# PaddlePaddle/PaddleScience

Hardware: AMD Instinct MI355X
Metric: collocation-points/sec (PDE residual+grad) (higher is better)
Workload: dtype f32; 1 GPU; Allen-Cahn 1D+t, MLP 2->64x4->1 tanh, 100k collocation pts per GPU, residual+MSE-mean+grad+Adam (BASELINE.json configs[1]); points_per_gpu=100000, parallelism=dp1, dp_step=fused tile kernel + tail kernel (sums, Adam, fragments)

## Files before the change

### paddlescience_amd/_lib.py

```python
from __future__ import annotations

import ctypes as C
import os
from typing import List, Optional, Sequence

MAX_IN, MAX_DIRS, MAX_OUT, MAX_HIDDEN, MAX_PROG, MAX_RES, MAX_AUX = 8, 4, 8, 16, 128, 8, 16

ACT = {"tanh": 0, "silu": 1, "sin": 2, "sigmoid": 3, "cos": 4, "gelu": 5, "swish": 6, "stan": 7, "relu": 8, "leaky_relu": 9,
       "elu": 10, "selu": 11, "identity": 12}
PARAM_ACTS = ("swish", "stan")
SIREN_W0 = 30.0
LINEAR_PLAIN, LINEAR_WEIGHT_NORM, LINEAR_RWF, LINEAR_FOURIER, LINEAR_BROADCAST = range(5)
LINEAR_PADDED = 100
EMBED_NONE, EMBED_PERIOD, EMBED_STREAMS = 0, 1, 2

(OP_LD_IN, OP_LD_U, OP_LD_AUX, OP_CONST, OP_ADD, OP_SUB, OP_MUL, OP_DIV, OP_NEG, OP_POW, OP_SIN, OP_COS,
 OP_TANH, OP_EXP, OP_LOG, OP_SQRT, OP_ABS, OP_SINH, OP_COSH, OP_TAN, OP_MAX, OP_MIN, OP_SIGN, OP_HEAVISIDE,
 OP_DETACH, OP_ASIN, OP_ACOS, OP_ATAN, OP_ATAN2, OP_ASINH, OP_ACOSH, OP_ATANH, OP_ERF, OP_LGAMMA, OP_CEIL, OP_FLOOR,
 OP_LD_PARAM, OP_COUNT) = range(38)
MAX_EPARAM = 8
MTL_MAX_LOSSES = 8
MTL_PCGRAD, MTL_GRAM_ONLY = 0, 1
STEP_KEEP_FRAGMENTS = 1


class MlpDesc(C.Structure):
    _fields_ = [
        ("d_raw", C.c_int32), ("n_hidden", C.c_int32), ("width", C.c_int32), ("d_out", C.c_int32),
        ("activation", C.c_int32), ("skip_connection", C.c_int32), ("n1", C.c_int32), ("n2", C.c_int32),
        ("embed", C.c_int32 * MAX_IN), ("omega", C.c_float * MAX_IN), ("dirs", (C.c_float * MAX_IN) * MAX_DIRS),
        ("act_scale", C.c_float), ("fourier_half", C.c_int32), ("n3", C.c_int32), ("n4", C.c_int32),
    ]


class SpectralDesc(C.Structure):
    _fields_ = [(n, C.c_int32) for n in ("batch", "c_in", "c_out", "h", "wf", "modes_x", "modes_y")]


class PwVirtual(C.Structure):
    _fields_ = [("mode", C.c_int32), ("K0", C.c_int32), ("x0", C.c_void_p), ("W0", C.c_void_p), ("b0", C.c_void_p)]


class ReduceSeg(C.Structure):
    _fields_ = [("partials", C.c_void_p), ("out", C.c_void_p), ("rows", C.c_int64), ("cols", C.c_int64), ("accumulate", C.c_int32)]


class LinearJob(C.Structure):
    _fields_ = [("kind", C.c_int32), ("fin", C.c_int32), ("fout", C.c_int32)] + [(n, C.c_void_p) for n in (
        "v", "g", "b", "W", "b_out", "gW", "gb", "gv", "gg", "gb_out")]


class ModMlpDesc(C.Structure):
    _fields_ = [(n, C.c_int32) for n in ("n_hidden", "width", "d_out", "activation")]


class SpinnGridDesc(C.Structure):
    _fields_ = [("n", C.c_int32 * 3), ("rank", C.c_int32), ("cu", C.c_float), ("cxx", C.c_float), ("cyy", C.c_float),
                ("czz", C.c_float), ("scale", C.c_float)]


SPINN_MAX_JET = 16


class SpinnJetDesc(C.Structure):
    _fields_ = [("n", C.c_int32 * 3), ("rank", C.c_int32), ("nq", C.c_int32), ("ord", (C.c_int32 * 3) * SPINN_MAX_JET)]


class PirateEmbedDesc(C.Structure):
    _fields_ = [("d_raw", C.c_int32), ("d0", C.c_int32), ("half", C.c_int32), ("n1", C.c_int32), ("n2", C.c_int32),
                ("embed", C.c_int32 * MAX_IN), ("omega", C.c_float * MAX_IN), ("dirs", (C.c_float * MAX_IN) * MAX_DIRS),
                ("N", C.c_int64), ("NP", C.c_int64)]


PIRATE_ACT, PIRATE_GATE, PIRATE_RES = 0, 1, 2


ONET_MAX_J = 3


class OnetHeadDesc(C.Structure):
    _fields_ = [("J", C.c_int32), ("p", C.c_int32), ("n_out", C.c_int32), ("n1", C.c_int32), ("n2", C.c_int32),
                ("act", C.c_int32), ("N", C.c_int64), ("NP", C.c_int64)]


class Fno1dLayerDesc(C.Structure):
    _fields_ = ([(k, C.c_void_p) for k in ("A1", "T", "A2", "X2", "bias", "ip_src", "ip_i0", "ip_t", "ia_src", "ia_first", "dact_v",
                                           "v", "out", "hw2", "hb2", "hy")]
                + [(k, C.c_int64) for k in ("a1_bs", "a2_rs", "a2_cs", "x2_bs", "ip_bs", "ia_bs", "dv_bs", "o_bs")]
                + [(k, C.c_int32) for k in ("ldt", "x2_ld", "x2_len", "ip_ld", "ia_ld", "dv_ld", "o_ld", "act", "B", "R", "K1", "K2",
                                            "Lc", "Lout")])


class LnoTriDesc(C.Structure):
    _fields_ = ([("n", C.c_int32 * 3), ("m", C.c_int32 * 3)] + [(k, C.c_int32) for k in (
        "nb", "ncp", "nc2", "C", "pair_cp", "pair_c2", "conj_t", "coef_b", "coef_cp", "coef_c2", "mult_conj")]
        + [("gscale", C.c_float)])


class Instr(C.Structure):
    _fields_ = [("op", C.c_int32), ("a", C.c_int32), ("b", C.c_int32), ("c", C.c_float)]


class Residual(C.Structure):
    _fields_ = [("value", C.c_int32), ("label", C.c_int32), ("weight", C.c_int32), ("area", C.c_int32),
                ("scale", C.c_float), ("kind", C.c_int32), ("scale_param", C.c_int32)]


class EpilogueDesc(C.Structure):
    _fields_ = [
        ("n_instr", C.c_int32), ("n_res", C.c_int32), ("n_streams", C.c_int32), ("n_in", C.c_int32),
        ("n_aux", C.c_int32), ("prog", Instr * MAX_PROG), ("res", Residual * MAX_RES),
    ]


class AdamArgs(C.Structure):
    _fields_ = [("m", C.c_void_p), ("v", C.c_void_p), ("lr", C.c_float), ("beta1", C.c_float), ("beta2", C.c_float),
                ("eps", C.c_float), ("grad_scale", C.c_float), ("step_t", C.c_int64)]


_HERE = os.path.dirname(os.path.abspath(__file__))
DEFAULT_LIB = os.environ.get("PPSCI_HIP_LIB") or os.path.join(_HERE, "libppsci_hip.so")
_lib: Optional[C.CDLL] = None
_injected = False

_SYMBOLS = {
    "ppsci_last_error": (C.c_char_p, []),
    "ppsci_is_device_build": (C.c_int, []),
    "ppsci_check_device": (C.c_int, []),
    "ppsci_linear_multi": (C.c_int, [C.c_int, C.POINTER(LinearJob), C.c_int, C.c_void_p]),
    "ppsci_reduce_rows_multi": (C.c_int, [C.c_int, C.POINTER(ReduceSeg), C.c_void_p]),
    "ppsci_reduce_rows_multi_adam": (C.c_int, [C.c_int, C.POINTER(ReduceSeg), C.c_int64, C.c_void_p, C.c_void_p, C.c_void_p,
                                               C.c_void_p, C.c_float, C.c_float, C.c_float, C.c_float, C.c_int64, C.c_float,
                                               C.c_void_p]),
    "ppsci_release_fragments": (None, [C.c_void_p]),
    "ppsci_set_max_grid": (None, [C.c_int]),
    "ppsci_set_wide_min_nb": (None, [C.c_int]),
    "ppsci_set_bwd_accum": (None, [C.c_int]),
    "ppsci_set_bwd_layerwise": (None, [C.c_int]),
    "ppsci_comm_unique_id": (C.c_int, [C.c_void_p]),
    "ppsci_comm_init": (C.c_int, [C.c_int, C.c_int, C.c_void_p]),
    "ppsci_comm_world_size": (C.c_int, []),
    "ppsci_allreduce_sum": (C.c_int, [C.c_void_p, C.c_int64, C.c_void_p]),
    "ppsci_allgather": (C.c_int, [C.c_void_p, C.c_void_p, C.c_int64, C.c_void_p]),
    "ppsci_comm_destroy": (C.c_int, []),
    "ppsci_param_count": (C.c_int64, [C.POINTER(MlpDesc)]),
    "ppsci_stash_bytes": (C.c_int64, [C.POINTER(MlpDesc), C.c_int64]),
    "ppsci_bwd_partial_rows": (C.c_int64, [C.POINTER(MlpDesc), C.c_int64]),
    "ppsci_bwd_workspace_bytes": (C.c_int64, [C.POINTER(MlpDesc), C.c_int64]),
    "ppsci_epilogue_partial_rows": (C.c_int64, [C.c_int64]),
    "ppsci_taylor_fwd": (C.c_int, [C.POINTER(MlpDesc), C.c_void_p, C.c_int64, C.POINTER(C.c_void_p), C.c_void_p,
                                   C.c_void_p, C.c_void_p]),
    "ppsci_epilogue": (C.c_int, [C.POINTER(EpilogueDesc), C.c_int64, C.POINTER(C.c_void_p), C.c_void_p,
                                 C.POINTER(C.c_void_p), C.c_void_p, C.c_void_p, C.c_void_p, C.c_void_p]),
    "ppsci_epilogue_losses": (C.c_int, [C.POINTER(EpilogueDesc), C.c_int64, C.POINTER(C.c_void_p), C.c_void_p,
                                        C.POINTER(C.c_void_p), C.c_void_p, C.c_void_p, C.c_void_p, C.c_void_p,
                                        C.c_void_p, C.c_void_p, C.c_void_p, C.c_void_p]),
    "ppsci_epilogue_params": (C.c_int, [C.POINTER(EpilogueDesc), C.c_int64, C.POINTER(C.c_void_p), C.c_void_p,
                                        C.POINTER(C.c_void_p), C.c_void_p, C.c_void_p, C.c_void_p, C.c_void_p,
                                        C.c_void_p, C.c_void_p]),
    "ppsci_taylor_bwd": (C.c_int, [C.POINTER(MlpDesc), C.c_void_p, C.c_int64, C.POINTER(C.c_void_p), C.c_void_p,
                                   C.c_void_p, C.c_void_p, C.c_void_p, C.c_void_p]),
    "ppsci_taylor_bwd_ws": (C.c_int, [C.POINTER(MlpDesc), C.c_void_p, C.c_int64, C.POINTER(C.c_void_p), C.c_void_p,
                                      C.c_void_p, C.c_void_p, C.c_int64, C.c_void_p, C.c_void_p]),
    "ppsci_dense_matvec": (C.c_int, [C.c_int64, C.c_int64, C.c_void_p, C.c_void_p, C.c_void_p, C.c_float, C.c_int, C.c_void_p,
                                     C.c_void_p]),
    "ppsci_csr_matvec": (C.c_int, [C.c_int64, C.c_int64, C.c_int64, C.c_void_p, C.c_void_p, C.c_void_p, C.c_void_p, C.c_void_p,
                                   C.c_float, C.c_void_p, C.c_void_p]),
    "ppsci_reduce_rows": (C.c_int, [C.c_void_p, C.c_int64, C.c_int64, C.c_void_p, C.c_int, C.c_void_p]),
    "ppsci_taylor_step_workspace_bytes": (C.c_int64, [C.POINTER(MlpDesc), C.POINTER(EpilogueDesc), C.c_int64]),
    "ppsci_taylor_step_kind": (C.c_int, [C.POINTER(MlpDesc), C.POINTER(EpilogueDesc), C.c_int64]),
    "ppsci_set_fused_step": (None, [C.c_int]),
    "ppsci_set_step_tail": (None, [C.c_int]),
    "ppsci_set_tail_split": (None, [C.c_int]),
    "ppsci_set_fast_program": (None, [C.c_int]),
    "ppsci_taylor_step_run_ex": (C.c_int, [C.c_void_p, C.c_int, C.POINTER(AdamArgs), C.c_void_p, C.c_int]),
    "ppsci_taylor_step_plan_apply": (C.c_int, [C.c_void_p, C.POINTER(AdamArgs), C.c_void_p]),
    "ppsci_set_static_program": (None, [C.c_int]),
    "ppsci_epilogue_predecode": (C.c_int, [C.POINTER(EpilogueDesc), C.POINTER(C.c_uint32), C.POINTER(C.c_int)]),
    "ppsci_taylor_step_plan_static": (C.c_int, [C.c_void_p, C.POINTER(C.c_char_p)]),
    "ppsci_set_fused_specialised": (None, [C.c_int]),
    "ppsci_taylor_step_plan_specialised": (C.c_int, [C.c_void_p]),
    "ppsci_set_fused_keep_planes": (None, [C.c_int]),
    "ppsci_taylor_step_plan_keep_planes": (C.c_int, [C.c_void_p]),
    "ppsci_taylor_step_plan": (C.c_void_p, [C.POINTER(MlpDesc), C.POINTER(EpilogueDesc), C.c_void_p, C.c_int64,
                                            C.POINTER(C.c_void_p), C.POINTER(C.c_void_p), C.c_void_p, C.c_void_p, C.c_void_p,
                                            C.c_void_p, C.c_void_p, C.c_int64, C.c_void_p, C.c_void_p]),
    "ppsci_taylor_step_run": (C.c_int, [C.c_void_p, C.c_int, C.POINTER(AdamArgs), C.c_void_p]),
    "ppsci_taylor_step_plan_set_scales": (C.c_int, [C.c_void_p, C.POINTER(EpilogueDesc)]),
    "ppsci_taylor_step_run_main": (C.c_int, [C.c_void_p, C.c_void_p]),
    "ppsci_taylor_step_plan_free": (None, [C.c_void_p]),
    "ppsci_taylor_step": (C.c_int, [C.POINTER(MlpDesc), C.POINTER(EpilogueDesc), C.c_void_p, C.c_int64, C.POINTER(C.c_void_p),
                                    C.POINTER(C.c_void_p), C.c_void_p, C.c_void_p, C.c_void_p, C.c_void_p, C.c_void_p,
                                    C.c_int64, C.c_void_p, C.c_void_p, C.c_int, C.POINTER(AdamArgs), C.c_void_p]),
    "ppsci_spectral_conv2d_fwd": (C.c_int, [C.POINTER(SpectralDesc), C.c_void_p, C.c_void_p, C.c_void_p, C.c_void_p,
                                            C.c_void_p]),
    "ppsci_spectral_conv2d_bwd": (C.c_int, [C.POINTER(SpectralDesc), C.c_void_p, C.c_void_p, C.c_void_p, C.c_void_p,
                                            C.c_void_p, C.c_void_p, C.c_void_p, C.c_void_p]),
    "ppsci_spectral_conv2d_bwd_real": (C.c_int, [C.POINTER(SpectralDesc), C.c_void_p, C.c_void_p, C.c_void_p, C.c_void_p,
                                                 C.c_void_p, C.c_void_p, C.c_void_p, C.c_float, C.c_int, C.c_void_p]),
    "ppsci_spectral_conv2d_fwd_scaled": (C.c_int, [C.POINTER(SpectralDesc), C.c_void_p, C.c_void_p, C.c_void_p, C.c_void_p,
                                                   C.c_float, C.c_int, C.c_void_p]),
    "ppsci_spectral_conv2d_bwd_real_scaled": (C.c_int, [C.POINTER(SpectralDesc), C.c_void_p, C.c_void_p, C.c_void_p,
                                                        C.c_void_p, C.c_void_p, C.c_void_p, C.c_void_p, C.c_float, C.c_int,
                                                        C.c_float, C.c_int, C.c_void_p]),
    "ppsci_dft2_kept_supported": (C.c_int, [C.c_int] * 4),
    "ppsci_dft2_kept_fwd": (C.c_int, [C.c_int] * 6 + [C.c_void_p] * 3),
    "ppsci_dft2_kept_inv": (C.c_int, [C.c_int] * 6 + [C.c_void_p] * 3),
    "ppsci_dft2_kept_inv_stats": (C.c_int, [C.c_int] * 6 + [C.c_void_p] * 3 + [C.c_int, C.c_void_p, C.c_void_p]),
    "ppsci_fno_tail_fwd_ex": (C.c_int, [C.c_int] * 5 + [C.c_float] + [C.c_void_p] * 9 + [C.c_int] * 5 + [C.c_void_p, C.c_void_p]),
    "ppsci_fno_tail_bwd_ex": (C.c_int, [C.c_int] * 5 + [C.c_void_p] * 13 + [C.c_int] * 4 + [C.c_void_p] * 3),
    "ppsci_spectral_conv2d_fwd_kept": (C.c_int, [C.POINTER(SpectralDesc)] + [C.c_void_p] * 4 + [C.c_float, C.c_void_p]),
    "ppsci_spectral_conv2d_inv_kept_ex": (C.c_int, [C.POINTER(SpectralDesc)] + [C.c_int] * 6 + [C.c_void_p, C.c_void_p, C.c_void_p, C.c_float,
                                                    C.c_void_p, C.c_void_p, C.c_void_p, C.c_void_p]),
    "ppsci_spectral_conv2d_inv_kept_supported": (C.c_int, [C.c_int] * 6),
    "ppsci_spectral_conv2d_inv_kept": (C.c_int, [C.POINTER(SpectralDesc), C.c_int, C.c_int, C.c_int, C.c_void_p, C.c_void_p,
                                                 C.c_void_p, C.c_float, C.c_void_p, C.c_void_p, C.c_void_p, C.c_void_p]),
    "ppsci_spectral_conv2d_bwd_kept": (C.c_int, [C.POINTER(SpectralDesc)] + [C.c_void_p] * 7 + [C.c_float, C.c_int, C.c_float,
                                                                                                 C.c_void_p]),
    "ppsci_fft2d_r2c": (C.c_int, [C.c_int, C.c_int, C.c_int, C.c_void_p, C.c_void_p, C.c_void_p]),
    "ppsci_fft2d_c2r": (C.c_int, [C.c_int, C.c_int, C.c_int, C.c_void_p, C.c_void_p, C.c_void_p]),
    "ppsci_pw_conv": (C.c_int, [C.c_int, C.c_int, C.c_int, C.c_int, C.c_void_p, C.c_void_p, C.c_int, C.c_void_p, C.c_void_p,
                                C.c_int, C.c_void_p, C.c_void_p, C.c_void_p]),
    "ppsci_pw_conv_v": (C.c_int, [C.c_int, C.c_int, C.c_int, C.c_int, C.c_void_p, C.POINTER(PwVirtual), C.c_void_p, C.c_int,
                                  C.c_void_p, C.c_void_p, C.POINTER(PwVirtual), C.c_int, C.c_void_p, C.c_void_p, C.c_void_p]),
    "ppsci_fno_proj_hidden_grad": (C.c_int, [C.c_int, C.c_int, C.c_int, C.c_int, C.c_void_p, C.c_void_p, C.c_void_p, C.c_void_p, C.c_void_p]),
    "ppsci_fno_lift0_wgrad": (C.c_int, [C.c_int, C.c_int, C.c_int, C.c_int, C.c_int, C.c_void_p, C.c_void_p, C.c_void_p, C.c_void_p,
                                        C.c_void_p, C.c_void_p, C.c_void_p, C.c_void_p, C.c_int64, C.c_void_p, C.c_int64, C.c_void_p]),
    "ppsci_pw_conv_wgrad_v": (C.c_int, [C.c_int, C.c_int, C.c_int, C.c_int, C.c_void_p, C.POINTER(PwVirtual), C.c_void_p,
                                        C.c_void_p, C.c_void_p, C.c_int64, C.c_void_p]),
    "ppsci_set_pw_pixels_per_lane": (None, [C.c_int]),
    "ppsci_pw_conv_wgrad_chunks": (C.c_int64, [C.c_int, C.c_int]),
    "ppsci_fno_lift0_wgrad_chunks": (C.c_int64, [C.c_int, C.c_int]),
    "ppsci_pw_conv_wgrad": (C.c_int, [C.c_int, C.c_int, C.c_int, C.c_int, C.c_void_p, C.c_void_p, C.c_void_p, C.c_void_p,
                                      C.c_void_p]),
    "ppsci_pad2d": (C.c_int, [C.c_int] * 8 + [C.c_void_p, C.c_void_p, C.c_void_p]),
    "ppsci_dft2_kept_from_supported": (C.c_int, [C.c_int] * 4),
    "ppsci_dft2_kept_fwd_from": (C.c_int, [C.c_int] * 7 + [C.c_void_p, C.c_void_p, C.c_void_p]),
    "ppsci_dft2_kept_inv_from": (C.c_int, [C.c_int] * 7 + [C.c_void_p, C.c_void_p, C.c_void_p]),
    "ppsci_sht_supported": (C.c_int, [C.c_int] * 4),
    "ppsci_sht_analysis": (C.c_int, [C.c_int] * 5 + [C.c_void_p] * 5),
    "ppsci_sht_synthesis": (C.c_int, [C.c_int] * 5 + [C.c_void_p] * 5),
    "ppsci_sht_contract": (C.c_int, [C.c_int] * 5 + [C.c_void_p] * 3 + [C.c_int, C.c_void_p, C.c_void_p]),
    "ppsci_sht_contract_wgrad": (C.c_int, [C.c_int] * 5 + [C.c_void_p] * 5),
    "ppsci_spectrum_resize": (C.c_int, [C.c_int] * 7 + [C.c_void_p, C.c_void_p, C.c_void_p]),
    "ppsci_resample2d_supported": (C.c_int, [C.c_int] * 4),
    "ppsci_resample2d": (C.c_int, [C.c_int] * 5 + [C.c_void_p] * 4 + [C.c_int, C.c_void_p]),
    "ppsci_field_loss_sums": (C.c_int, [C.c_int] * 4 + [C.c_float, C.c_float, C.c_int, C.c_int] + [C.c_void_p] * 4),
    "ppsci_field_loss_finish": (C.c_int, [C.c_int, C.c_int, C.c_float, C.c_float] + [C.c_void_p] * 4),
    "ppsci_field_loss_adjoint": (C.c_int, [C.c_int] * 4 + [C.c_float, C.c_float, C.c_int, C.c_int] + [C.c_void_p] * 5),
    "ppsci_tanh_fwd": (C.c_int, [C.c_int64, C.c_void_p, C.c_void_p, C.c_void_p]),
    "ppsci_tanh_bwd": (C.c_int, [C.c_int64, C.c_void_p, C.c_void_p, C.c_void_p, C.c_int, C.c_void_p]),
    "ppsci_fno_tail_fwd": (C.c_int, [C.c_int, C.c_int, C.c_int, C.c_int, C.c_int, C.c_float, C.c_void_p, C.c_void_p,
                                     C.c_void_p, C.c_void_p, C.c_void_p, C.c_void_p, C.c_void_p, C.c_void_p, C.c_void_p,
                                     C.c_void_p]),
    "ppsci_fno_tail_bwd": (C.c_int, [C.c_int, C.c_int, C.c_int, C.c_int, C.c_int, C.c_void_p, C.c_void_p, C.c_void_p,
                                     C.c_void_p, C.c_void_p, C.c_void_p, C.c_void_p, C.c_void_p, C.c_void_p, C.c_void_p,
                                     C.c_void_p, C.c_void_p, C.c_void_p, C.c_void_p]),
    "ppsci_modmlp_param_count": (C.c_int64, [C.POINTER(ModMlpDesc)]),
    "ppsci_modmlp_bwd_rows": (C.c_int64, [C.POINTER(ModMlpDesc), C.c_int64]),
    "ppsci_modmlp_bwd_parts_supported": (C.c_int, [C.POINTER(ModMlpDesc), C.POINTER(SpinnGridDesc)]),
    "ppsci_modmlp_bwd_batch_parts": (C.c_int, [C.POINTER(ModMlpDesc), C.POINTER(SpinnGridDesc), C.POINTER(C.c_void_p),
                                               C.POINTER(C.c_void_p), C.c_void_p, C.POINTER(C.c_void_p), C.POINTER(C.c_void_p),
                                               C.c_int64, C.c_void_p]),
    "ppsci_set_modmlp_tile": (None, [C.c_int]),
    "ppsci_modmlp_stash_floats": (C.c_int64, [C.POINTER(ModMlpDesc), C.c_int64]),
    "ppsci_modmlp_fwd": (C.c_int, [C.POINTER(ModMlpDesc), C.c_void_p, C.c_int64, C.c_void_p, C.c_void_p, C.c_void_p,
                                   C.c_void_p]),
    "ppsci_modmlp_bwd": (C.c_int, [C.POINTER(ModMlpDesc), C.c_void_p, C.c_int64, C.c_void_p, C.c_void_p, C.c_void_p,
                                   C.c_void_p, C.c_void_p]),
    "ppsci_modmlp_fwd_batch": (C.c_int, [C.POINTER(ModMlpDesc), C.c_int, C.POINTER(C.c_void_p), C.POINTER(C.c_int64),
                                         C.POINTER(C.c_void_p), C.POINTER(C.c_void_p), C.POINTER(C.c_void_p), C.c_void_p]),
    "ppsci_modmlp_bwd_batch": (C.c_int, [C.POINTER(ModMlpDesc), C.c_int, C.POINTER(C.c_void_p), C.POINTER(C.c_int64),
                                         C.POINTER(C.c_void_p), C.POINTER(C.c_void_p), C.POINTER(C.c_void_p),
                                         C.POINTER(C.c_void_p), C.c_int64, C.c_void_p]),
    "ppsci_pirate_embed_fwd": (C.c_int, [C.POINTER(PirateEmbedDesc), C.POINTER(C.c_void_p), C.c_void_p, C.c_void_p, C.c_void_p]),
    "ppsci_pirate_embed_chunks": (C.c_int64, [C.c_int64]),
    "ppsci_pirate_embed_bwd": (C.c_int, [C.POINTER(PirateEmbedDesc), C.POINTER(C.c_void_p), C.c_void_p, C.c_void_p, C.c_void_p,
                                         C.c_void_p]),
    "ppsci_pirate_act_chunks": (C.c_int64, [C.c_int64]),
    "ppsci_pirate_act_fwd": (C.c_int, [C.c_int, C.c_int, C.c_int, C.c_int64, C.c_int64, C.c_int, C.c_int] + [C.c_void_p] * 8),
    "ppsci_pirate_act_bwd": (C.c_int, [C.c_int, C.c_int, C.c_int, C.c_int64, C.c_int64, C.c_int, C.c_int] + [C.c_void_p] * 14),
    "ppsci_pirate_out_fwd": (C.c_int, [C.c_int, C.c_int, C.c_int64, C.c_int64, C.c_void_p, C.c_void_p, C.c_void_p, C.c_void_p]),
    "ppsci_pirate_out_bwd": (C.c_int, [C.c_int, C.c_int, C.c_int64, C.c_int64, C.c_void_p, C.c_void_p, C.c_void_p]),
    "ppsci_onet_pack": (C.c_int, [C.c_int, C.c_int64, C.c_int64, C.c_void_p, C.c_void_p, C.c_void_p]),
    "ppsci_onet_head_chunks": (C.c_int64, [C.c_int64]),
    "ppsci_onet_head_fwd": (C.c_int, [C.POINTER(OnetHeadDesc), C.c_void_p, C.c_void_p, C.POINTER(C.c_void_p),
                                      C.POINTER(C.c_void_p), C.c_void_p, C.c_void_p, C.c_void_p, C.c_void_p]),
    "ppsci_onet_head_bwd": (C.c_int, [C.POINTER(OnetHeadDesc), C.c_void_p, C.c_void_p, C.POINTER(C.c_void_p),
                                      C.POINTER(C.c_void_p), C.c_void_p, C.c_void_p, C.c_void_p, C.POINTER(C.c_void_p)]
                            + [C.c_void_p] * 5),
    "ppsci_lno_supported": (C.c_int, [C.c_int] * 6),
    "ppsci_lno_tables": (C.c_int, [C.c_int, C.POINTER(C.c_int), C.POINTER(C.c_int)] + [C.POINTER(C.c_void_p)] * 6 + [C.c_void_p]),
    "ppsci_lno_dft3": (C.c_int, [C.c_int] * 5 + [C.c_void_p, C.c_int, C.c_void_p, C.c_int, C.c_int, C.c_int, C.c_float, C.c_void_p,
                                 C.c_void_p, C.c_int, C.c_int, C.c_int, C.c_float, C.c_int, C.c_void_p, C.c_void_p]),
    "ppsci_lno_analysis": (C.c_int, [C.POINTER(LnoTriDesc), C.c_void_p, C.c_int, C.POINTER(C.c_void_p), C.c_void_p, C.c_void_p,
                                     C.c_void_p, C.c_void_p, C.c_int, C.POINTER(C.c_void_p), C.POINTER(C.c_void_p),
                                     C.POINTER(C.c_void_p), C.c_int, C.c_void_p]),
    "ppsci_lno_synthesis": (C.c_int, [C.POINTER(LnoTriDesc), C.POINTER(C.c_void_p), C.c_void_p, C.c_void_p, C.c_void_p, C.c_int,
                                      C.c_int, C.c_float, C.c_void_p, C.c_void_p]),
    "ppsci_lno_channel_sum": (C.c_int, [C.c_int] * 3 + [C.c_void_p] * 3 + [C.c_float, C.c_void_p, C.c_void_p]),
    "ppsci_lno_rho_grad": (C.c_int, [C.c_int] * 3 + [C.c_void_p] * 6),
    "ppsci_lno_hbar": (C.c_int, [C.c_int] * 3 + [C.c_void_p, C.c_void_p, C.c_float, C.c_void_p, C.c_void_p]),
    "ppsci_lno_inorm_fwd": (C.c_int, [C.c_int, C.c_int, C.c_float] + [C.c_void_p] * 4),
    "ppsci_lno_inorm_bwd": (C.c_int, [C.c_int, C.c_int] + [C.c_void_p] * 6),
    "ppsci_lno_point_rows": (C.c_int64, [C.c_int64]),
    "ppsci_lno_lift_fwd": (C.c_int, [C.c_int] * 7 + [C.c_void_p] * 5),
    "ppsci_lno_lift_bwd": (C.c_int, [C.c_int] * 7 + [C.c_void_p] * 6),
    "ppsci_lno_head_supported": (C.c_int, [C.c_int, C.c_int]),
    "ppsci_lno_head_fwd": (C.c_int, [C.c_int] * 5 + [C.c_void_p] * 10),
    "ppsci_lno_head_bwd": (C.c_int, [C.c_int] * 5 + [C.c_void_p] * 12),
    "ppsci_fno1d_point_rows": (C.c_int64, [C.c_int64]),
    "ppsci_fno1d_lift_fwd": (C.c_int, [C.c_int] * 5 + [C.c_void_p] * 5),
    "ppsci_fno1d_lift_bwd": (C.c_int, [C.c_int] * 5 + [C.c_void_p] * 6),
    "ppsci_fno1d_analysis": (C.c_int, [C.c_int] * 4 + [C.c_int64] + [C.c_void_p] * 4),
    "ppsci_fno1d_mix": (C.c_int, [C.c_int] * 5 + [C.c_void_p] * 6),
    "ppsci_fno1d_mix_wgrad": (C.c_int, [C.c_int] * 3 + [C.c_void_p] * 5),
    "ppsci_fno1d_layer_supported": (C.c_int, [C.c_int] * 3),
    "ppsci_fno1d_layer": (C.c_int, [C.POINTER(Fno1dLayerDesc), C.c_void_p]),
    "ppsci_fno1d_wgrad": (C.c_int, [C.c_int] * 6 + [C.c_void_p, C.c_int64, C.c_int, C.c_void_p, C.c_int64, C.c_int, C.c_void_p, C.c_void_p]),
    "ppsci_fno1d_head_pre": (C.c_int, [C.c_int] * 3 + [C.c_void_p] * 6),
    "ppsci_spinn_grid_partial_rows": (C.c_int64, [C.POINTER(SpinnGridDesc)]),
    "ppsci_spinn_grid_fwd": (C.c_int, [C.POINTER(SpinnGridDesc), C.c_void_p, C.c_void_p, C.c_void_p, C.c_void_p,
                                       C.c_void_p, C.c_void_p, C.c_void_p, C.c_void_p]),
    "ppsci_spinn_grid_bwd_scratch_floats": (C.c_int64, [C.POINTER(SpinnGridDesc)]),
    "ppsci_spinn_grid_bwd": (C.c_int, [C.POINTER(SpinnGridDesc), C.c_void_p, C.c_void_p, C.c_void_p, C.c_void_p,
                                       C.c_void_p, C.c_void_p, C.c_void_p, C.c_void_p, C.c_void_p]),
    "ppsci_spinn_jet_fwd": (C.c_int, [C.POINTER(SpinnJetDesc)] + [C.c_void_p] * 5),
    "ppsci_spinn_jet_scratch_floats": (C.c_int64, [C.POINTER(SpinnJetDesc)]),
    "ppsci_spinn_jet_bwd": (C.c_int, [C.POINTER(SpinnJetDesc)] + [C.c_void_p] * 9),
    "ppsci_adam_step": (C.c_int, [C.c_int64, C.c_void_p, C.c_void_p, C.c_void_p, C.c_void_p, C.c_float, C.c_float,
                                  C.c_float, C.c_float, C.c_int64, C.c_float, C.c_void_p]),
    "ppsci_grad_surgery_workspace_bytes": (C.c_int64, [C.c_int, C.c_int64]),
    "ppsci_grad_surgery": (C.c_int, [C.c_int, C.c_int64, C.c_void_p, C.c_int64, C.POINTER(C.c_int32), C.c_int, C.c_void_p,
                                     C.c_void_p, C.c_void_p, C.c_void_p, C.c_int64, C.c_void_p]),
    "ppsci_grad_combine": (C.c_int, [C.c_int, C.c_int64, C.c_void_p, C.c_int64, C.c_void_p, C.POINTER(C.c_float), C.c_void_p,
                                     C.c_void_p, C.POINTER(AdamArgs), C.c_void_p]),
    "ppsci_optim_step": (C.c_int, [C.c_int, C.c_int64, C.c_void_p, C.c_void_p, C.c_void_p, C.c_void_p, C.c_void_p,
                                   C.POINTER(C.c_float), C.c_int, C.c_void_p]),
    "ppsci_causal_weights": (C.c_int, [C.c_int64, C.c_int, C.c_float, C.c_void_p, C.c_void_p, C.c_void_p, C.c_void_p,
                                       C.c_void_p, C.c_void_p, C.c_void_p]),
    "ppsci_linear_materialize": (C.c_int, [C.c_int, C.c_int, C.c_int, C.c_void_p, C.c_void_p, C.c_void_p, C.c_void_p,
                                           C.c_void_p, C.c_void_p]),
    "ppsci_linear_pad": (C.c_int, [C.c_int, C.c_int, C.c_int, C.c_int, C.c_void_p, C.c_void_p, C.c_void_p, C.c_void_p,
                                   C.c_void_p]),
    "ppsci_linear_unpad": (C.c_int, [C.c_int, C.c_int, C.c_int, C.c_int, C.c_void_p, C.c_void_p, C.c_void_p, C.c_void_p,
                                     C.c_void_p]),
    "ppsci_linear_pullback": (C.c_int, [C.c_int, C.c_int, C.c_int, C.c_void_p, C.c_void_p, C.c_void_p, C.c_void_p,
                                        C.c_void_p, C.c_void_p, C.c_void_p, C.c_void_p]),
}

EXPORTED_SYMBOLS = tuple(_SYMBOLS)


def _bind(path: str) -> C.CDLL:
    lib_ = C.CDLL(path)
    for name, (res, args) in _SYMBOLS.items():
        fn = getattr(lib_, name)
        fn.restype = res
        fn.argtypes = args
    return lib_


def lib() -> C.CDLL:
    global _lib
    if _lib is None:
        if not os.path.exists(DEFAULT_LIB):
            raise RuntimeError(
                f"{DEFAULT_LIB} not found: build it with `python -c 'import __graft_entry__ as g; g.build()'` "
                "(hipcc --offload-arch=gfx950). paddlescience_amd has no CPU fallback."
            )
        l = _bind(DEFAULT_LIB)
        if l.ppsci_is_device_build() != 1:
            raise RuntimeError(f"{DEFAULT_LIB} is not a gfx950 device build")
        import torch

        if torch.cuda.is_available() and l.ppsci_check_device() != 0:
            raise RuntimeError(l.ppsci_last_error().decode())
        _lib = l
    return _lib


def _inject_for_tests(path: Optional[str]) -> None:
    global _lib, _injected
    _lib = _bind(path) if path else None
    _injected = path is not None


def is_emulated() -> bool:
    return _injected


def check(rc: int) -> None:
    if rc != 0:
        msg = lib().ppsci_last_error()
        raise RuntimeError(f"libppsci_hip error {rc}: {msg.decode() if msg else ''}")


def ptr_array(ptrs: Sequence[int]):
    arr = (C.c_void_p * max(1, len(ptrs)))()
    for i, p in enumerate(ptrs):
        arr[i] = p
    return arr


def make_mlp_desc(d_raw: int, n_hidden: int, width: int, d_out: int, activation: str, skip_connection: bool,
                  dirs: Sequence[Sequence[float]], n2: int, embed: Optional[Sequence[int]] = None,
                  omega: Optional[Sequence[float]] = None, fourier_half: int = 0, n3: int = 0, n4: int = 0) -> MlpDesc:
    d = MlpDesc()
    d.n3, d.n4 = int(n3), int(n4)
    d.fourier_half = int(fourier_half)
    d.d_raw, d.n_hidden, d.width, d.d_out = d_raw, n_hidden, width, d_out
    if activation == "siren":
        activation, d.act_scale = "sin", SIREN_W0
    if activation not in ACT:
        raise NotImplementedError(f"activation {activation!r} has no HIP kernel (supported: {sorted(ACT)})")
    d.activation = ACT[activation]
    d.skip_connection = 1 if skip_connection else 0
    d.n1, d.n2 = len(dirs), n2
    if len(dirs) > MAX_DIRS:
        raise NotImplementedError(f"at most {MAX_DIRS} derivative directions per launch, got {len(dirs)}")
    for i, row in enumerate(dirs):
        for j, v in enumerate(row):
            d.dirs[i][j] = float(v)
    for j in range(d_raw):
        d.embed[j] = int(embed[j]) if embed is not None else 0
        d.omega[j] = float(omega[j]) if omega is not None else 0.0
    return d
```

### paddlescience_amd/csrc/wgrad_reduce.hip

```cpp
#include "taylor_tile.h"

#include <string.h>

struct WRedArgs {
  const float* wpart;
  float* tmp;
  float* row;
  const float* small;
  float* tmp_small;
  int nsmall_rows, psmall, nbs;
  int m, d0;
  ppsci_derived q;
  int L, H, ntiles, nchunks, nb4;
  long long per_tile;
  long long tmp_stride, small_stride, loss_stride;
  ppsci_wred_extras x;
};

__global__ void __launch_bounds__(256) wgrad_reduce1_kernel(WRedArgs a) {
  if ((int)blockIdx.x >= a.nchunks * a.nb4) {
    const int bid = (int)blockIdx.x - a.nchunks * a.nb4;
    const int chunk = bid / a.nbs;
    const int j = (bid - chunk * a.nbs) * 256 + threadIdx.x;
    if (j >= a.psmall) return;
    const int r0 = (int)((long long)a.nsmall_rows * chunk / a.nchunks);
    const int r1 = (int)((long long)a.nsmall_rows * (chunk + 1) / a.nchunks);
    float v = 0.f;
#pragma unroll 8
    for (int r = r0; r < r1; ++r) v += a.small[(long long)r * a.psmall + j];
    a.tmp_small[(long long)chunk * a.psmall + j] = v;
    return;
  }
  const int chunk = blockIdx.x / a.nb4;
  const long long j4 = (long long)(blockIdx.x - chunk * a.nb4) * 256 + threadIdx.x;
  if (j4 * 4 >= a.per_tile) return;
  const int t0 = (int)((long long)a.ntiles * chunk / a.nchunks);
  const int t1 = (int)((long long)a.ntiles * (chunk + 1) / a.nchunks);
  f32x4 s = (f32x4){0.f, 0.f, 0.f, 0.f};
  const f32x4* src = (const f32x4*)a.wpart + j4;
  const long long stride4 = a.per_tile / 4;
#pragma unroll 8
  for (int t = t0; t < t1; ++t) s += __builtin_nontemporal_load(&src[(long long)t * stride4]);
  ((f32x4*)a.tmp)[(long long)chunk * stride4 + j4] = s;
}

__global__ void __launch_bounds__(256) wgrad_reduce2_kernel(WRedArgs a) {
  if ((int)blockIdx.x >= (a.q.P + 255) / 256) {
    __shared__ float red[4];
    for (int k = 0; k < a.x.n_res; ++k) {
      float v = 0.f;
#pragma unroll 4
      for (int r = threadIdx.x; r < a.x.loss_nrows; r += 256) v += a.x.loss_rows[(long long)r * a.loss_stride + k];
#pragma unroll
      for (int off = 32; off >= 1; off >>= 1) v += __shfl_xor(v, off, 64);
      if ((threadIdx.x & 63) == 0) red[threadIdx.x >> 6] = v;
      __syncthreads();
      if (threadIdx.x == 0) a.x.loss_out[k] = (red[0] + red[1]) + (red[2] + red[3]);
      __syncthreads();
    }
    return;
  }
  const int idx = blockIdx.x * 256 + threadIdx.x;
  if (idx >= a.q.P) return;
  float v = 0.f;
  bool hidden = false;
  for (int l = 1; l < a.L; ++l) {
    const int off = a.q.offW[l];
    if (idx >= off && idx < off + a.H * a.H) {
      hidden = true;
      const int e = idx - off;
      const int in = e / a.H, out = e - in * a.H;
      const int NB = a.q.NB, HP = a.q.HP;
      const long long j = (long long)(l - 1) * HP * HP +
                          ((long long)((in >> 4) * NB + (out >> 4)) * 64 + 16 * ((in & 15) >> 2) + (out & 15)) * 4 + (in & 3);
      float v4[4] = {0.f, 0.f, 0.f, 0.f};
#pragma unroll 4
      for (int c = 0; c < a.nchunks; c += 4) {
#pragma unroll
        for (int u = 0; u < 4; ++u) {
          const int cu = c + u < a.nchunks ? c + u : a.nchunks - 1;
          const float t = a.tmp[(long long)cu * a.tmp_stride + j];
          v4[u] += c + u < a.nchunks ? t : 0.f;
        }
      }
      v = (v4[0] + v4[1]) + (v4[2] + v4[3]);
    }
  }
  if (!hidden) {
    const int H = a.H, L = a.L;
    int ci;
    if (idx >= a.q.offB[L]) ci = (a.d0 + L + a.m) * H + (idx - a.q.offB[L]);
    else if (idx >= a.q.offW[L]) ci = (a.d0 + L) * H + (idx - a.q.offW[L]);
    else if (idx < a.q.offW[0] + a.d0 * H) ci = idx - a.q.offW[0];
    else {
      int l = 0;
      while (l + 1 < L && idx >= a.q.offW[l + 1]) ++l;
      ci = a.d0 * H + l * H + (idx - a.q.offB[l]);
    }
    float v4[4] = {0.f, 0.f, 0.f, 0.f};
#pragma unroll 4
    for (int c = 0; c < a.nchunks; c += 4) {
#pragma unroll
      for (int u = 0; u < 4; ++u) {
        const int cu = c + u < a.nchunks ? c + u : a.nchunks - 1;
        const float t = a.tmp_small[(long long)cu * a.small_stride + ci];
        v4[u] += c + u < a.nchunks ? t : 0.f;
      }
    }
    v = (v4[0] + v4[1]) + (v4[2] + v4[3]);
  }
  if (a.x.accumulate) v += a.row[idx];
  a.row[idx] = v;
  if (a.x.p != nullptr) {
    const float g = v * a.x.grad_scale;
    const float mm = a.x.beta1 * a.x.m[idx] + (1.f - a.x.beta1) * g;
    const float vv = a.x.beta2 * a.x.v[idx] + (1.f - a.x.beta2) * g * g;
    a.x.m[idx] = mm;
    a.x.v[idx] = vv;
    a.x.p[idx] = a.x.p[idx] - a.x.lr_t * (mm / (sqrtf(vv) + a.x.eps_t));
  }
}

int ppsci_wgrad_reduce_chunks(const ppsci_mlp_desc& d, const ppsci_derived& q, int nrows, const float* rows, long long rowlen,
                              long long off_small, long long off_loss, float* row, const ppsci_wred_extras& x0, void* stream) {
  WRedArgs a;
  memset(&a, 0, sizeof(a));
  a.x = x0;
  a.x.loss_rows = x0.loss_out ? rows + off_loss : nullptr;
  a.x.loss_nrows = nrows;
  a.psmall = ppsci_small_params(d, q);
  a.m = d.d_out;
  a.d0 = q.d0;
  a.tmp = (float*)rows;
  a.tmp_small = (float*)rows + off_small;
  a.row = row;
  a.q = q;
  a.L = d.n_hidden;
  a.H = d.width;
  a.nchunks = nrows;
  a.per_tile = (long long)(d.n_hidden - 1) * q.HP * q.HP;
  a.tmp_stride = a.small_stride = a.loss_stride = rowlen;
  PPSCI_LAUNCH(wgrad_reduce2_kernel, WRedArgs, (q.P + 255) / 256 + (a.x.loss_rows != nullptr ? 1 : 0), 256, 0, stream, a);
  if (PPSCI_LAST_LAUNCH_ERROR() != 0) {
    ppsci_set_error("wgrad_reduce2: launch failed");
    return PPSCI_E_LAUNCH;
  }
  return PPSCI_OK;
}

int ppsci_wgrad_reduce(const ppsci_mlp_desc& d, const ppsci_derived& q, int ntiles, const float* wpart, float* tmp,
                       const float* small_rows, int nsmall_rows, float* tmp_small, float* row, void* stream) {
  ppsci_wred_extras none;
  memset(&none, 0, sizeof(none));
  return ppsci_wgrad_reduce_ex(d, q, ntiles, wpart, tmp, small_rows, nsmall_rows, tmp_small, row, none, stream);
}

int ppsci_wgrad_reduce_ex(const ppsci_mlp_desc& d, const ppsci_derived& q, int ntiles, const float* wpart, float* tmp,
                          const float* small_rows, int nsmall_rows, float* tmp_small, float* row, const ppsci_wred_extras& x,
                          void* stream) {
  WRedArgs a;
  a.x = x;
  a.small = small_rows;
  a.tmp_small = tmp_small;
  a.nsmall_rows = nsmall_rows;
  a.psmall = ppsci_small_params(d, q);
  a.nbs = (a.psmall + 255) / 256;
  a.m = d.d_out;
  a.d0 = q.d0;
  a.wpart = wpart;
  a.tmp = tmp;
  a.row = row;
  a.q = q;
  a.L = d.n_hidden;
  a.H = d.width;
  a.ntiles = ntiles;
  a.nchunks = ntiles < PPSCI_WRED_CHUNKS ? ntiles : PPSCI_WRED_CHUNKS;
  if (a.nchunks < 1) a.nchunks = 1;
  a.per_tile = (long long)(d.n_hidden - 1) * q.HP * q.HP;
  a.tmp_stride = a.per_tile, a.small_stride = a.psmall, a.loss_stride = x.n_res;
  a.nb4 = a.per_tile > 0 ? (int)((a.per_tile / 4 + 255) / 256) : 0;
  {
    PPSCI_LAUNCH(wgrad_reduce1_kernel, WRedArgs, a.nchunks * (a.nb4 + a.nbs), 256, 0, stream, a);
    int e = PPSCI_LAST_LAUNCH_ERROR();
    if (e != 0) {
      ppsci_set_error("wgrad_reduce1: launch failed (hip error %d)", e);
      return PPSCI_E_LAUNCH;
    }
  }
  PPSCI_LAUNCH(wgrad_reduce2_kernel, WRedArgs, (q.P + 255) / 256 + (x.loss_rows != nullptr ? 1 : 0), 256, 0, stream, a);
  int e = PPSCI_LAST_LAUNCH_ERROR();
  if (e != 0) {
    ppsci_set_error("wgrad_reduce2: launch failed (hip error %d)", e);
    return PPSCI_E_LAUNCH;
  }
  return PPSCI_OK;
}

struct WTailArgs {
  const float* rows_w;
  const float* rows_s;
  float* row;
  u32x4* frag;
  ppsci_derived q;
  int L, H, m, d0, nrows, psmall, nblk, nsmall;
  long long per_tile, loss_stride;
  ppsci_wred_extras x;
};

__device__ __forceinline__ float wtail_adam(const ppsci_wred_extras& x, int idx, float gsum) {
  const float g = gsum * x.grad_scale;
  const float mm = x.beta1 * x.m[idx] + (1.f - x.beta1) * g;
  const float vv = x.beta2 * x.v[idx] + (1.f - x.beta2) * g * g;
  x.m[idx] = mm;
  x.v[idx] = vv;
  const float pn = x.p[idx] - x.lr_t * (mm / (sqrtf(vv) + x.eps_t));
  x.p[idx] = pn;
  return pn;
}

__device__ __forceinline__ int wtail_small_index(const WTailArgs& a, int ci) {
  const int H = a.H, L = a.L;
  if (ci < a.d0 * H) return a.q.offW[0] + ci;
  if (ci < (a.d0 + L) * H) {
    const int lb = (ci - a.d0 * H) / H;
    return a.q.offB[lb] + (ci - a.d0 * H - lb * H);
  }
  if (ci < (a.d0 + L + a.m) * H) return a.q.offW[L] + (ci - (a.d0 + L) * H);
  return a.q.offB[L] + (ci - (a.d0 + L + a.m) * H);
}

__global__ void __launch_bounds__(1024) wgrad_tail_kernel(WTailArgs a) {
  __shared__ f32x4 red[16][64];
  __shared__ float tile[16][17];
  const int tid = threadIdx.x, lane = tid & 63, rg = tid >> 6;
  const int b = blockIdx.x;
  if (b < a.nblk) {
    const long long stride4 = a.per_tile / 4;
    const f32x4* src = (const f32x4*)a.rows_w + (long long)b * 64 + lane;
    f32x4 acc[4];
#pragma unroll
    for (int u = 0; u < 4; ++u) acc[u] = (f32x4){0.f, 0.f, 0.f, 0.f};
#pragma unroll 2
    for (int r0 = rg; r0 < a.nrows; r0 += 64) {
#pragma unroll
      for (int u = 0; u < 4; ++u) {
        const int r = r0 + 16 * u;
        const f32x4 v = __builtin_nontemporal_load(&src[(long long)(r < a.nrows ? r : a.nrows - 1) * stride4]);
        acc[u] += r < a.nrows ? v : (f32x4){0.f, 0.f, 0.f, 0.f};
      }
    }
    red[rg][lane] = (acc[0] + acc[1]) + (acc[2] + acc[3]);
    __syncthreads();
    if (rg != 0) return;
    f32x4 tot = red[0][lane];
#pragma unroll
    for (int w = 1; w < 16; ++w) tot += red[w][lane];
    const int NB = a.q.NB, NKP = NB / 2;
    const int l = b / (NB * NB), blk = b - l * NB * NB, ib = blk / NB, ob = blk - ib * NB;
    const int g = lane >> 4, c = lane & 15;
    const int in0 = 16 * ib + 4 * g, out = 16 * ob + c;
    f32x4 pn = (f32x4){0.f, 0.f, 0.f, 0.f};
#pragma unroll
    for (int r = 0; r < 4; ++r) {
      if (in0 + r < a.H && out < a.H) {
        const int idx = a.q.offW[l + 1] + (in0 + r) * a.H + out;
        float v = tot[r];
        if (a.x.accumulate) v += a.row[idx];
        a.row[idx] = v;
        if (a.x.p != nullptr) pn[r] = wtail_adam(a.x, idx, v);
      }
    }
    if (a.x.p == nullptr || a.frag == nullptr) return;
    const long long per_layer = (long long)NB * NKP * 3 * 64;
    {
      const ppsci_split4 sp = ppsci_split(pn);
      u32x2* dst = (u32x2*)(a.frag + (long long)l * per_layer + (long long)((ob * NKP + (ib >> 1)) * 3) * 64 + lane) + (ib & 1);
#pragma unroll
      for (int p = 0; p < 3; ++p) dst[(long long)p * 64 * 2] = sp.p[p];
    }
#pragma unroll
    for (int r = 0; r < 4; ++r) tile[4 * g + r][c] = pn[r];
    ppsci_wave_sync();
    f32x4 pt;
#pragma unroll
    for (int r = 0; r < 4; ++r) pt[r] = tile[c][4 * g + r];
    {
      const ppsci_split4 sp = ppsci_split(pt);
      u32x2* dst = (u32x2*)(a.frag + (long long)(a.L - 1 + l) * per_layer + (long long)((ib * NKP + (ob >> 1)) * 3) * 64 + lane) + (ob & 1);
#pragma unroll
      for (int p = 0; p < 3; ++p) dst[(long long)p * 64 * 2] = sp.p[p];
    }
    return;
  }
  if (b < a.nblk + a.nsmall) {
    float* redf = (float*)red;
    const int ci = (b - a.nblk) * 64 + lane;
    const int cc = ci < a.psmall ? ci : 0;
    float acc[4] = {0.f, 0.f, 0.f, 0.f};
#pragma unroll 2
    for (int r0 = rg; r0 < a.nrows; r0 += 64) {
#pragma unroll
      for (int u = 0; u < 4; ++u) {
        const int r = r0 + 16 * u;
        const float v = a.rows_s[(long long)(r < a.nrows ? r : a.nrows - 1) * a.psmall + cc];
        acc[u] += r < a.nrows ? v : 0.f;
      }
    }
    redf[rg * 64 + lane] = (acc[0] + acc[1]) + (acc[2] + acc[3]);
    __syncthreads();
    if (rg != 0 || ci >= a.psmall) return;
    float v = redf[lane];
#pragma unroll
    for (int w = 1; w < 16; ++w) v += redf[w * 64 + lane];
    const int idx = wtail_small_index(a, ci);
    if (a.x.accumulate) v += a.row[idx];
    a.row[idx] = v;
    if (a.x.p != nullptr) wtail_adam(a.x, idx, v);
    return;
  }
  float* redf = (float*)red;
  for (int k = 0; k < a.x.n_res; ++k) {
    float v = 0.f;
#pragma unroll 4
    for (int r = tid; r < a.x.loss_nrows; r += 1024) v += a.x.loss_rows[(long long)r * a.loss_stride + k];
#pragma unroll
    for (int off = 32; off >= 1; off >>= 1) v += __shfl_xor(v, off, 64);
    if (lane == 0) redf[rg] = v;
    __syncthreads();
    if (tid == 0) {
      float s = redf[0];
      for (int w = 1; w < 16; ++w) s += redf[w];
      a.x.loss_out[k] = s;
    }
    __syncthreads();
  }
}

__global__ void __launch_bounds__(256) wgrad_tail_split_kernel(WTailArgs a) {
  __shared__ f32x4 red[16][16];
  __shared__ float tile[4][17];
  const int tid = threadIdx.x, c = tid & 15, rg = tid >> 4;
  const int b = blockIdx.x;
  if (b < 4 * a.nblk) {
    const int blk_l = b >> 2, g = b & 3, lane = 16 * g + c;
    const long long stride4 = a.per_tile / 4;
    const f32x4* src = (const f32x4*)a.rows_w + (long long)blk_l * 64 + lane;
    f32x4 acc[4];
#pragma unroll
    for (int u = 0; u < 4; ++u) acc[u] = (f32x4){0.f, 0.f, 0.f, 0.f};
#pragma unroll 4
    for (int r0 = rg; r0 < a.nrows; r0 += 64) {
#pragma unroll
      for (int u = 0; u < 4; ++u) {
        const int r = r0 + 16 * u;
        const f32x4 v = __builtin_nontemporal_load(&src[(long long)(r < a.nrows ? r : a.nrows - 1) * stride4]);
        acc[u] += r < a.nrows ? v : (f32x4){0.f, 0.f, 0.f, 0.f};
      }
    }
    red[rg][c] = (acc[0] + acc[1]) + (acc[2] + acc[3]);
    __syncthreads();
    if (tid >= 64) return;
    const bool own = tid < 16;
    const int NB = a.q.NB, NKP = NB / 2;
    const int l = blk_l / (NB * NB), blk = blk_l - l * NB * NB, ib = blk / NB, ob = blk - ib * NB;
    f32x4 pn = (f32x4){0.f, 0.f, 0.f, 0.f};
    if (own) {
      f32x4 tot = red[0][c];
#pragma unroll
      for (int w = 1; w < 16; ++w) tot += red[w][c];
      const int in0 = 16 * ib + 4 * g, out = 16 * ob + c;
#pragma unroll
      for (int r = 0; r < 4; ++r) {
        if (in0 + r < a.H && out < a.H) {
          const int idx = a.q.offW[l + 1] + (in0 + r) * a.H + out;
          float v = tot[r];
          if (a.x.accumulate) v += a.row[idx];
          a.row[idx] = v;
          if (a.x.p != nullptr) pn[r] = wtail_adam(a.x, idx, v);
        }
      }
    }
    if (a.x.p == nullptr || a.frag == nullptr) return;
    const long long per_layer = (long long)NB * NKP * 3 * 64;
    if (own) {
      const ppsci_split4 sp = ppsci_split(pn);
      u32x2* dst = (u32x2*)(a.frag + (long long)l * per_layer + (long long)((ob * NKP + (ib >> 1)) * 3) * 64 + lane) + (ib & 1);
#pragma unroll
      for (int p = 0; p < 3; ++p) dst[(long long)p * 64 * 2] = sp.p[p];
#pragma unroll
      for (int r = 0; r < 4; ++r) tile[r][c] = pn[r];
    }
    ppsci_wave_sync();
    if (own) {
      const int gd = c >> 2, i = c & 3, laned = 16 * gd + 4 * g + i;
      f32x4 pt;
#pragma unroll
      for (int r = 0; r < 4; ++r) pt[r] = tile[i][4 * gd + r];
      const ppsci_split4 sp = ppsci_split(pt);
      u32x2* dst = (u32x2*)(a.frag + (long long)(a.L - 1 + l) * per_layer + (long long)((ib * NKP + (ob >> 1)) * 3) * 64 + laned) + (ob & 1);
#pragma unroll
      for (int p = 0; p < 3; ++p) dst[(long long)p * 64 * 2] = sp.p[p];
    }
    return;
  }
  if (b < 4 * a.nblk + a.nsmall) {
    float* redf = (float*)red;
    const int ci = (b - 4 * a.nblk) * 16 + c;
    const int cc = ci < a.psmall ? ci : 0;
    float acc[4] = {0.f, 0.f, 0.f, 0.f};
#pragma unroll 4
    for (int r0 = rg; r0 < a.nrows; r0 += 64) {
#pragma unroll
      for (int u = 0; u < 4; ++u) {
        const int r = r0 + 16 * u;
        const float v = a.rows_s[(long long)(r < a.nrows ? r : a.nrows - 1) * a.psmall + cc];
        acc[u] += r < a.nrows ? v : 0.f;
      }
    }
    redf[rg * 16 + c] = (acc[0] + acc[1]) + (acc[2] + acc[3]);
    __syncthreads();
    if (rg != 0 || ci >= a.psmall) return;
    float v = redf[c];
#pragma unroll
    for (int w = 1; w < 16; ++w) v += redf[w * 16 + c];
    const int idx = wtail_small_index(a, ci);
    if (a.x.accumulate) v += a.row[idx];
    a.row[idx] = v;
    if (a.x.p != nullptr) wtail_adam(a.x, idx, v);
    return;
  }
  float* redf = (float*)red;
  const int lane = tid & 63, wv = tid >> 6;
  for (int k = 0; k < a.x.n_res; ++k) {
    for (int pass = 0; pass < 4; ++pass) {
      float v = 0.f;
#pragma unroll 4
      for (int r = 256 * pass + tid; r < a.x.loss_nrows; r += 1024) v += a.x.loss_rows[(long long)r * a.loss_stride + k];
#pragma unroll
      for (int off = 32; off >= 1; off >>= 1) v += __shfl_xor(v, off, 64);
      if (lane == 0) redf[4 * pass + wv] = v;
    }
    __syncthreads();
    if (tid == 0) {
      float s = redf[0];
      for (int w = 1; w < 16; ++w) s += redf[w];
      a.x.loss_out[k] = s;
    }
    __syncthreads();
  }
}

#ifndef PPSCI_TAIL_SPLIT_DEFAULT
#define PPSCI_TAIL_SPLIT_DEFAULT 0
#endif
static int g_tail_split = PPSCI_TAIL_SPLIT_DEFAULT;
extern "C" void ppsci_set_tail_split(int n) { g_tail_split = n == 1 ? 1 : (n == 0 ? PPSCI_TAIL_SPLIT_DEFAULT : 0); }

int ppsci_wgrad_tail(const ppsci_mlp_desc& d, const ppsci_derived& q, int nrows, const float* rows_w, const float* rows_s,
                     float* row, const ppsci_wred_extras& x, void* frag, void* stream) {
  WTailArgs a;
  memset(&a, 0, sizeof(a));
  a.rows_w = rows_w;
  a.rows_s = rows_s;
  a.row = row;
  a.frag = (u32x4*)frag;
  a.q = q;
  a.L = d.n_hidden;
  a.H = d.width;
  a.m = d.d_out;
  a.d0 = q.d0;
  a.nrows = nrows;
  a.psmall = ppsci_small_params(d, q);
  a.nblk = (d.n_hidden - 1) * q.NB * q.NB;
  a.per_tile = (long long)(d.n_hidden - 1) * q.HP * q.HP;
  a.loss_stride = x.n_res;
  a.x = x;
  const int nloss = x.loss_rows != nullptr ? 1 : 0;
  if (g_tail_split == 1) {
    a.nsmall = (a.psmall + 63) / 64;
    PPSCI_LAUNCH(wgrad_tail_kernel, WTailArgs, a.nblk + a.nsmall + nloss, 1024, 0, stream, a);
  } else {
    a.nsmall = (a.psmall + 15) / 16;
    PPSCI_LAUNCH(wgrad_tail_split_kernel, WTailArgs, 4 * a.nblk + a.nsmall + nloss, 256, 0, stream, a);
  }
  if (PPSCI_LAST_LAUNCH_ERROR() != 0) {
    ppsci_set_error("wgrad_tail: launch failed");
    return PPSCI_E_LAUNCH;
  }
  return PPSCI_OK;
}
```

Baseline: 495.5 million points/s.

## Add row-wave tail reduction kernel and make it the default

Adds a new tail kernel that reduces per-tile weight-gradient rows with 1024-thread blocks. Each of 16 waves covers interleaved rows, with 8 loads in flight per thread and cross-wave reduction through shared memory. Adam and fragment writes are fused as before. The aim is more memory-level parallelism when summing partial gradients over many tile rows. The trade-off is higher register and shared-memory use and extra block synchronisation in a small tail kernel.

```diff
diff --git a/paddlescience_amd/_lib.py b/paddlescience_amd/_lib.py
--- a/paddlescience_amd/_lib.py
+++ b/paddlescience_amd/_lib.py
@@ -22,6 +22,7 @@
 MTL_MAX_LOSSES = 8
 MTL_PCGRAD, MTL_GRAM_ONLY = 0, 1
 STEP_KEEP_FRAGMENTS = 1
+TAIL_DEFAULT, TAIL_UNSPLIT, TAIL_SPLIT, TAIL_ROWWAVE = 0, 1, 2, 3
 
 
 class MlpDesc(C.Structure):
diff --git a/paddlescience_amd/csrc/wgrad_reduce.hip b/paddlescience_amd/csrc/wgrad_reduce.hip
--- a/paddlescience_amd/csrc/wgrad_reduce.hip
+++ b/paddlescience_amd/csrc/wgrad_reduce.hip
@@ -450,11 +450,190 @@
   }
 }
 
+__device__ __forceinline__ float wtail_adam_pre(const ppsci_wred_extras& x, int idx, float gsum, float m0, float v0, float p0) {
+  const float g = gsum * x.grad_scale;
+  const float mm = x.beta1 * m0 + (1.f - x.beta1) * g;
+  const float vv = x.beta2 * v0 + (1.f - x.beta2) * g * g;
+  x.m[idx] = mm;
+  x.v[idx] = vv;
+  const float pn = p0 - x.lr_t * (mm / (sqrtf(vv) + x.eps_t));
+  x.p[idx] = pn;
+  return pn;
+}
+
+__device__ __forceinline__ int wtail_small_index_flat(const WTailArgs& a, int ci) {
+  const int H = a.H, L = a.L;
+  if (ci < a.d0 * H) return a.q.offW[0] + ci;
+  if (ci < (a.d0 + L) * H) {
+    const int lb = (ci - a.d0 * H) / H;
+    return (lb == 0 ? a.q.offB[0] : a.q.offB[1] + (lb - 1) * (H * H + H)) + (ci - a.d0 * H - lb * H);
+  }
+  if (ci < (a.d0 + L + a.m) * H) return a.q.offW[L] + (ci - (a.d0 + L) * H);
+  return a.q.offB[L] + (ci - (a.d0 + L + a.m) * H);
+}
+
+__global__ void __launch_bounds__(1024) wgrad_tail_rowwave_kernel(WTailArgs a) {
+  __shared__ f32x4 red[16][16];
+  __shared__ float tile[4][17];
+  const int tid = threadIdx.x, lane = tid & 63, c = lane & 15, u = lane >> 4, rg = tid >> 6;
+  const int b = blockIdx.x;
+  const bool own = tid < 16;
+  if (b < 4 * a.nblk) {
+    const int blk_l = b >> 2, g = b & 3;
+    const int NB = a.q.NB, NKP = NB / 2;
+    const int l = blk_l / (NB * NB), blk = blk_l - l * NB * NB, ib = blk / NB, ob = blk - ib * NB;
+    const int in0 = 16 * ib + 4 * g, out = 16 * ob + c;
+    const long long stride4 = a.per_tile / 4;
+    const f32x4* src = (const f32x4*)a.rows_w + (long long)blk_l * 64 + 16 * g + c;
+    const int nr = a.nrows, rb = rg + 16 * u;
+    f32x4 v[8];
+#pragma unroll
+    for (int k = 0; k < 8; ++k) v[k] = (f32x4){0.f, 0.f, 0.f, 0.f};
+    if (nr > 0) {
+#pragma unroll
+      for (int k = 0; k < 8; ++k) v[k] = __builtin_nontemporal_load(&src[(long long)(rb + 64 * k < nr ? rb + 64 * k : nr - 1) * stride4]);
+    }
+    float g0[4] = {0.f, 0.f, 0.f, 0.f}, m0[4] = {0.f, 0.f, 0.f, 0.f}, v0[4] = {0.f, 0.f, 0.f, 0.f}, p0[4] = {0.f, 0.f, 0.f, 0.f};
+    if (own) {
+      int idx[4];
+#pragma unroll
+      for (int r = 0; r < 4; ++r) idx[r] = a.q.offW[l + 1] + (in0 + r < a.H && out < a.H ? (in0 + r) * a.H + out : 0);
+      if (a.x.accumulate) {
+#pragma unroll
+        for (int r = 0; r < 4; ++r) g0[r] = a.row[idx[r]];
+      }
+      if (a.x.p != nullptr) {
+#pragma unroll
+        for (int r = 0; r < 4; ++r) m0[r] = a.x.m[idx[r]], v0[r] = a.x.v[idx[r]], p0[r] = a.x.p[idx[r]];
+      }
+    }
+#pragma unroll
+    for (int k = 0; k < 8; ++k) PPSCI_OPAQUE(v[k]);
+    f32x4 acc = (f32x4){0.f, 0.f, 0.f, 0.f};
+#pragma unroll
+    for (int k = 0; k < 8; ++k) acc += rb + 64 * k < nr ? v[k] : (f32x4){0.f, 0.f, 0.f, 0.f};
+    for (int r0 = rb + 512; r0 < nr; r0 += 512) {
+#pragma unroll
+      for (int k = 0; k < 8; ++k) {
+        const int r = r0 + 64 * k;
+        const f32x4 w = __builtin_nontemporal_load(&src[(long long)(r < nr ? r : nr - 1) * stride4]);
+        acc += r < nr ? w : (f32x4){0.f, 0.f, 0.f, 0.f};
+      }
+    }
+    f32x4 part;
+#pragma unroll
+    for (int i = 0; i < 4; ++i) {
+      const float s = acc[i] + __shfl_xor(acc[i], 16, 64);
+      part[i] = s + __shfl_xor(s, 32, 64);
+    }
+    if (u == 0) red[rg][c] = part;
+    __syncthreads();
+    if (tid >= 64) return;
+    f32x4 pn = (f32x4){0.f, 0.f, 0.f, 0.f};
+    if (own) {
+      f32x4 tot = red[0][c];
+#pragma unroll
+      for (int w = 1; w < 16; ++w) tot += red[w][c];
+#pragma unroll
+      for (int r = 0; r < 4; ++r) {
+        if (in0 + r < a.H && out < a.H) {
+          const int idx = a.q.offW[l + 1] + (in0 + r) * a.H + out;
+          float v = tot[r];
+          if (a.x.accumulate) v += g0[r];
+          a.row[idx] = v;
+          if (a.x.p != nullptr) pn[r] = wtail_adam_pre(a.x, idx, v, m0[r], v0[r], p0[r]);
+        }
+      }
+    }
+    if (a.x.p == nullptr || a.frag == nullptr) return;
+    const long long per_layer = (long long)NB * NKP * 3 * 64;
+    if (own) {
+      const ppsci_split4 sp = ppsci_split(pn);
+      u32x2* dst = (u32x2*)(a.frag + (long long)l * per_layer + (long long)((ob * NKP + (ib >> 1)) * 3) * 64 + 16 * g + c) + (ib & 1);
+#pragma unroll
+      for (int p = 0; p < 3; ++p) dst[(long long)p * 64 * 2] = sp.p[p];
+#pragma unroll
+      for (int r = 0; r < 4; ++r) tile[r][c] = pn[r];
+    }
+    ppsci_wave_sync();
+    if (own) {
+      const int gd = c >> 2, i = c & 3, laned = 16 * gd + 4 * g + i;
+      f32x4 pt;
+#pragma unroll
+      for (int r = 0; r < 4; ++r) pt[r] = tile[i][4 * gd + r];
+      const ppsci_split4 sp = ppsci_split(pt);
+      u32x2* dst = (u32x2*)(a.frag + (long long)(a.L - 1 + l) * per_layer + (long long)((ib * NKP + (ob >> 1)) * 3) * 64 + laned) + (ob & 1);
+#pragma unroll
+      for (int p = 0; p < 3; ++p) dst[(long long)p * 64 * 2] = sp.p[p];
+    }
+    return;
+  }
+  if (b < 4 * a.nblk + a.nsmall) {
+    float* redf = (float*)red;
+    const int ci = (b - 4 * a.nblk) * 16 + c;
+    const int cc = ci < a.psmall ? ci : 0;
+    const bool mine = own && ci < a.psmall;
+    const int idx = wtail_small_index_flat(a, cc);
+    const int nr = a.nrows, rb = rg + 16 * u;
+    float v[8] = {0.f, 0.f, 0.f, 0.f, 0.f, 0.f, 0.f, 0.f};
+    if (nr > 0) {
+#pragma unroll
+      for (int k = 0; k < 8; ++k) v[k] = a.rows_s[(long long)(rb + 64 * k < nr ? rb + 64 * k : nr - 1) * a.psmall + cc];
+    }
+    float g0 = 0.f, m0 = 0.f, v0 = 0.f, p0 = 0.f;
+    if (mine) {
+      if (a.x.accumulate) g0 = a.row[idx];
+      if (a.x.p != nullptr) m0 = a.x.m[idx], v0 = a.x.v[idx], p0 = a.x.p[idx];
+    }
+#pragma unroll
+    for (int k = 0; k < 8; ++k) PPSCI_OPAQUE(v[k]);
+    float acc = 0.f;
+#pragma unroll
+    for (int k = 0; k < 8; ++k) acc += rb + 64 * k < nr ? v[k] : 0.f;
+    for (int r0 = rb + 512; r0 < nr; r0 += 512) {
+#pragma unroll
+      for (int k = 0; k < 8; ++k) {
+        const int r = r0 + 64 * k;
+        const float w = a.rows_s[(long long)(r < nr ? r : nr - 1) * a.psmall + cc];
+        acc += r < nr ? w : 0.f;
+      }
+    }
+    const float s = acc + __shfl_xor(acc, 16, 64);
+    const float part = s + __shfl_xor(s, 32, 64);
+    if (u == 0) redf[rg * 16 + c] = part;
+    __syncthreads();
+    if (!mine) return;
+    float tot = redf[c];
+#pragma unroll
+    for (int w = 1; w < 16; ++w) tot += redf[w * 16 + c];
+    if (a.x.accumulate) tot += g0;
+    a.row[idx] = tot;
+    if (a.x.p != nullptr) wtail_adam_pre(a.x, idx, tot, m0, v0, p0);
+    return;
+  }
+  float* redf = (float*)red;
+  for (int k = 0; k < a.x.n_res; ++k) {
+    float v = 0.f;
+#pragma unroll 4
+    for (int r = tid; r < a.x.loss_nrows; r += 1024) v += a.x.loss_rows[(long long)r * a.loss_stride + k];
+#pragma unroll
+    for (int off = 32; off >= 1; off >>= 1) v += __shfl_xor(v, off, 64);
+    if (lane == 0) redf[rg] = v;
+    __syncthreads();
+    if (tid == 0) {
+      float s = redf[0];
+      for (int w = 1; w < 16; ++w) s += redf[w];
+      a.x.loss_out[k] = s;
+    }
+    __syncthreads();
+  }
+}
+
 #ifndef PPSCI_TAIL_SPLIT_DEFAULT
-#define PPSCI_TAIL_SPLIT_DEFAULT 0
+#define PPSCI_TAIL_SPLIT_DEFAULT 3
 #endif
 static int g_tail_split = PPSCI_TAIL_SPLIT_DEFAULT;
-extern "C" void ppsci_set_tail_split(int n) { g_tail_split = n == 1 ? 1 : (n == 0 ? PPSCI_TAIL_SPLIT_DEFAULT : 0); }
+extern "C" void ppsci_set_tail_split(int n) { g_tail_split = n == 1 || n == 3 ? n : (n == 0 ? PPSCI_TAIL_SPLIT_DEFAULT : 0); }
 
 int ppsci_wgrad_tail(const ppsci_mlp_desc& d, const ppsci_derived& q, int nrows, const float* rows_w, const float* rows_s,
                      float* row, const ppsci_wred_extras& x, void* frag, void* stream) {
@@ -479,6 +658,9 @@
   if (g_tail_split == 1) {
     a.nsmall = (a.psmall + 63) / 64;
     PPSCI_LAUNCH(wgrad_tail_kernel, WTailArgs, a.nblk + a.nsmall + nloss, 1024, 0, stream, a);
+  } else if (g_tail_split == 3) {
+    a.nsmall = (a.psmall + 15) / 16;
+    PPSCI_LAUNCH(wgrad_tail_rowwave_kernel, WTailArgs, 4 * a.nblk + a.nsmall + nloss, 1024, 0, stream, a);
   } else {
     a.nsmall = (a.psmall + 15) / 16;
     PPSCI_LAUNCH(wgrad_tail_split_kernel, WTailArgs, 4 * a.nblk + a.nsmall + nloss, 256, 0, stream, a);
```

Result: no change. 491.0 million points/s, median of 2 (-0.9%).
